# rust-bio/rust-bio

Measured on NVIDIA H100. Metric: GCUPS, higher is better.
Workload: dtype int32

## Files before the change

### rust_bio_b200/csrc/b2a_kernels.cuh

```cuda
#pragma once
#include <cuda_runtime.h>

#include "b2a_common.cuh"

namespace b2a {

struct PackParams {
  const Block* blocks;
  const uint32_t* order;
  const uint8_t* blob;
  const uint64_t* x_off;
  const uint32_t* x_len;
  const uint64_t* y_off;
  const uint32_t* y_len;
  const uint8_t* codemap;
  uint8_t* seq;
  uint32_t* bad_symbol;
  int32_t G;
  int32_t mapped;
};

__global__ void __launch_bounds__(256) pack_kernel(const PackParams prm) {
  __shared__ uint8_t cmap[256];
  __shared__ uint64_t s_off[64];
  __shared__ uint32_t s_len[64];
  cmap[threadIdx.x] = prm.codemap[threadIdx.x];
  const Block blk = prm.blocks[blockIdx.x];
  if (threadIdx.x < 64) {
    const uint32_t pair = threadIdx.x & 31u;
    const bool isy = threadIdx.x >= 32;
    uint64_t off = 0;
    uint32_t len = 0;
    if (pair < blk.npairs) {
      const uint32_t orig = prm.order[blk.first + pair];
      off = isy ? prm.y_off[orig] : prm.x_off[orig];
      len = isy ? prm.y_len[orig] : prm.x_len[orig];
    }
    s_off[threadIdx.x] = off;
    s_len[threadIdx.x] = len;
  }
  __syncthreads();
  const int G = prm.G, P = 32 / G;
  uint32_t* out = reinterpret_cast<uint32_t*>(prm.seq + blk.seq_off);
  const uint32_t xtot = blk.xwords * 32, ytot = blk.ywords * 32;
  for (uint32_t k = threadIdx.x; k < xtot + ytot; k += blockDim.x) {
    const bool isy = k >= xtot;
    const uint32_t kk = isy ? k - xtot : k;
    const uint32_t words = isy ? blk.ywords : blk.xwords;
    const uint32_t pair = kk / words, w = kk % words;
    uint32_t val = 0;
    {
      const uint64_t off = s_off[pair + (isy ? 32u : 0u)];
      const uint32_t len = s_len[pair + (isy ? 32u : 0u)];
      const uint32_t pos0 = w * 4;
      if (pos0 < len) {
        uint32_t raw;
        const uint32_t have = len - pos0 < 4 ? len - pos0 : 4;
        if (((off & 3ull) == 0) && have == 4) {
          raw = *reinterpret_cast<const uint32_t*>(prm.blob + off + pos0);
        } else {
          raw = 0;
          for (uint32_t b = 0; b < have; ++b) raw |= (uint32_t)prm.blob[off + pos0 + b] << (8 * b);
        }
#pragma unroll
        for (int b = 0; b < 4; ++b) {
          if ((uint32_t)b < have) {
            uint32_t code = cmap[(raw >> (8 * b)) & 0xFFu];
            if (prm.mapped && code == 0xFFu) {
              *prm.bad_symbol = 1u;
              code = 0;
            }
            val |= code << (8 * b);
          }
        }
      }
    }
    const uint32_t sub = pair / P, p = pair % P;
    out[(isy ? (size_t)G * blk.xwords * P : 0) + ((size_t)sub * words + w) * P + p] = val;
  }
}

__global__ void __launch_bounds__(256) symbols_kernel(const uint8_t* __restrict__ blob, uint64_t n,
                                                      uint32_t* __restrict__ flags) {
  __shared__ uint32_t seen[256];
  seen[threadIdx.x] = 0;
  __syncthreads();
  const uint64_t stride = (uint64_t)gridDim.x * blockDim.x;
  for (uint64_t i = blockIdx.x * (uint64_t)blockDim.x + threadIdx.x; i < n; i += stride) seen[blob[i]] = 1u;
  __syncthreads();
  if (seen[threadIdx.x]) flags[threadIdx.x] = 1u;
}

__global__ void gather_ops_kernel(const uint8_t* __restrict__ scratch,
                                  const uint64_t* __restrict__ ops_src,
                                  const uint64_t* __restrict__ ops_off, uint8_t* __restrict__ dense,
                                  uint64_t n_pairs) {
  const uint64_t warp = (blockIdx.x * (uint64_t)blockDim.x + threadIdx.x) >> 5;
  const uint32_t lane = threadIdx.x & 31;
  if (warp >= n_pairs) return;
  const uint64_t lo = ops_off[warp], n = ops_off[warp + 1] - lo;
  const uint8_t* src = scratch + ops_src[warp];
  for (uint64_t k = lane; k < n; k += 32) dense[lo + k] = src[k];
}

__global__ void __launch_bounds__(1024) scan_small_kernel(const uint32_t* __restrict__ n_ops, uint64_t* __restrict__ off,
                                                          uint32_t n_pairs) {
  __shared__ uint32_t wsum[64][32];
  __shared__ uint32_t round_tot[64];
  __shared__ uint64_t round_base[65];
  const uint32_t lane = threadIdx.x & 31u, w = threadIdx.x >> 5;
  const uint32_t rounds = (n_pairs + 1023u) >> 10;
  auto warp_inc = [&](uint32_t v) {
    for (int d = 1; d < 32; d <<= 1) {
      const uint32_t t = __shfl_up_sync(0xffffffffu, v, d);
      if (lane >= (uint32_t)d) v += t;
    }
    return v;
  };
  for (uint32_t k = 0; k < rounds; ++k) {
    const uint32_t i = (k << 10) + threadIdx.x;
    const uint32_t inc = warp_inc(i < n_pairs ? n_ops[i] : 0u);
    if (lane == 31) wsum[k][w] = inc;
  }
  __syncthreads();
  for (uint32_t k = w; k < rounds; k += 32) {
    const uint32_t ws = wsum[k][lane], wi = warp_inc(ws);
    wsum[k][lane] = wi - ws;
    if (lane == 31) round_tot[k] = wi;
  }
  __syncthreads();
  if (w == 0) {
    uint64_t carry = 0;
    for (uint32_t k0 = 0; k0 < rounds; k0 += 32) {
      const uint32_t k = k0 + lane;
      const uint64_t v = k < rounds ? (uint64_t)round_tot[k] : 0ull;
      uint64_t inc = v;
      for (int d = 1; d < 32; d <<= 1) {
        const uint64_t t = __shfl_up_sync(0xffffffffu, inc, d);
        if (lane >= (uint32_t)d) inc += t;
      }
      if (k < rounds) round_base[k] = carry + inc - v;
      carry += __shfl_sync(0xffffffffu, inc, 31);
    }
    if (lane == 0) round_base[rounds] = carry;
  }
  __syncthreads();
  for (uint32_t k = 0; k < rounds; ++k) {
    const uint32_t i = (k << 10) + threadIdx.x;
    const uint32_t v = i < n_pairs ? n_ops[i] : 0u;
    const uint32_t inc = warp_inc(v);
    if (i < n_pairs) off[i] = round_base[k] + wsum[k][w] + (inc - v);
  }
  if (threadIdx.x == 0) off[n_pairs] = round_base[rounds];
}

__global__ void widen_kernel(const uint32_t* __restrict__ n_ops, uint64_t* __restrict__ out,
                             uint64_t n_pairs) {
  const uint64_t i = blockIdx.x * (uint64_t)blockDim.x + threadIdx.x;
  if (i <= n_pairs) out[i] = i < n_pairs ? n_ops[i] : 0;
}

__global__ void records_kernel(const int32_t* score, const uint32_t* xstart, const uint32_t* xend,
                               const uint32_t* ystart, const uint32_t* yend, const uint32_t* n_ops,
                               const uint32_t* clip_len, const uint8_t* scratch,
                               const uint64_t* ops_src, uint8_t* records, uint32_t stride,
                               uint64_t n_pairs) {
  const uint64_t warp = (blockIdx.x * (uint64_t)blockDim.x + threadIdx.x) >> 5;
  const uint32_t lane = threadIdx.x & 31;
  if (warp >= n_pairs) return;
  uint8_t* rec = records + warp * stride;
  uint32_t* head = reinterpret_cast<uint32_t*>(rec);
  const uint32_t n = n_ops[warp];
  if (lane == 0) {
    head[0] = (uint32_t)score[warp];
    head[1] = xstart[warp];
    head[2] = xend[warp];
    head[3] = ystart[warp];
    head[4] = yend[warp];
    head[5] = n;
  }
  if (lane < 4) head[6 + lane] = clip_len[4 * warp + lane];
  const uint8_t* src = scratch + ops_src[warp];
  for (uint32_t k = lane; k < stride - 40; k += 32) rec[40 + k] = k < n ? src[k] : 0;
}

}
```

Before: 852.7.

## Transpose pack_kernel output through a padded shared-memory tile for coalesced stores

```diff
diff --git a/rust_bio_b200/csrc/b2a_kernels.cuh b/rust_bio_b200/csrc/b2a_kernels.cuh
--- a/rust_bio_b200/csrc/b2a_kernels.cuh
+++ b/rust_bio_b200/csrc/b2a_kernels.cuh
@@ -20,10 +20,40 @@
   int32_t mapped;
 };
 
+__device__ __forceinline__ uint32_t pack_word(const PackParams& prm, const uint8_t* cmap, const uint64_t off,
+                                              const uint32_t len, const uint32_t w) {
+  uint32_t val = 0;
+  const uint32_t pos0 = w * 4;
+  if (pos0 < len) {
+    uint32_t raw;
+    const uint32_t have = len - pos0 < 4 ? len - pos0 : 4;
+    if (((off & 3ull) == 0) && have == 4) {
+      raw = *reinterpret_cast<const uint32_t*>(prm.blob + off + pos0);
+    } else {
+      raw = 0;
+      for (uint32_t b = 0; b < have; ++b) raw |= (uint32_t)prm.blob[off + pos0 + b] << (8 * b);
+    }
+#pragma unroll
+    for (int b = 0; b < 4; ++b) {
+      if ((uint32_t)b < have) {
+        uint32_t code = cmap[(raw >> (8 * b)) & 0xFFu];
+        if (prm.mapped && code == 0xFFu) {
+          *prm.bad_symbol = 1u;
+          code = 0;
+        }
+        val |= code << (8 * b);
+      }
+    }
+  }
+  return val;
+}
+
+constexpr int PACK_CW_LOG = 6, PACK_CW = 1 << PACK_CW_LOG;
 __global__ void __launch_bounds__(256) pack_kernel(const PackParams prm) {
   __shared__ uint8_t cmap[256];
   __shared__ uint64_t s_off[64];
   __shared__ uint32_t s_len[64];
+  __shared__ uint32_t tile[PACK_CW * 33];
   cmap[threadIdx.x] = prm.codemap[threadIdx.x];
   const Block blk = prm.blocks[blockIdx.x];
   if (threadIdx.x < 64) {
@@ -41,42 +71,23 @@
   }
   __syncthreads();
   const int G = prm.G, P = 32 / G;
-  uint32_t* out = reinterpret_cast<uint32_t*>(prm.seq + blk.seq_off);
-  const uint32_t xtot = blk.xwords * 32, ytot = blk.ywords * 32;
-  for (uint32_t k = threadIdx.x; k < xtot + ytot; k += blockDim.x) {
-    const bool isy = k >= xtot;
-    const uint32_t kk = isy ? k - xtot : k;
-    const uint32_t words = isy ? blk.ywords : blk.xwords;
-    const uint32_t pair = kk / words, w = kk % words;
-    uint32_t val = 0;
-    {
-      const uint64_t off = s_off[pair + (isy ? 32u : 0u)];
-      const uint32_t len = s_len[pair + (isy ? 32u : 0u)];
-      const uint32_t pos0 = w * 4;
-      if (pos0 < len) {
-        uint32_t raw;
-        const uint32_t have = len - pos0 < 4 ? len - pos0 : 4;
-        if (((off & 3ull) == 0) && have == 4) {
-          raw = *reinterpret_cast<const uint32_t*>(prm.blob + off + pos0);
-        } else {
-          raw = 0;
-          for (uint32_t b = 0; b < have; ++b) raw |= (uint32_t)prm.blob[off + pos0 + b] << (8 * b);
-        }
-#pragma unroll
-        for (int b = 0; b < 4; ++b) {
-          if ((uint32_t)b < have) {
-            uint32_t code = cmap[(raw >> (8 * b)) & 0xFFu];
-            if (prm.mapped && code == 0xFFu) {
-              *prm.bad_symbol = 1u;
-              code = 0;
-            }
-            val |= code << (8 * b);
-          }
-        }
+  const int plog = 31 - __clz(P);
+  for (int side = 0; side < 2; ++side) {
+    const uint32_t words = side ? blk.ywords : blk.xwords;
+    uint32_t* out = reinterpret_cast<uint32_t*>(prm.seq + blk.seq_off) + (side ? (size_t)G * blk.xwords * P : 0);
+    for (uint32_t w0 = 0; w0 < words; w0 += PACK_CW) {
+      const uint32_t cw = words - w0 < (uint32_t)PACK_CW ? words - w0 : (uint32_t)PACK_CW;
+      for (uint32_t k = threadIdx.x; k < 32u * PACK_CW; k += blockDim.x) {
+        const uint32_t pair = k >> PACK_CW_LOG, wl = k & (PACK_CW - 1);
+        if (wl < cw) tile[wl * 33 + pair] = pack_word(prm, cmap, s_off[32 * side + pair], s_len[32 * side + pair], w0 + wl);
       }
+      __syncthreads();
+      for (uint32_t k = threadIdx.x; k < 32u * PACK_CW; k += blockDim.x) {
+        const uint32_t p = k & (P - 1), wl = (k >> plog) & (PACK_CW - 1), sub = k >> (plog + PACK_CW_LOG);
+        if (wl < cw) out[((size_t)sub * words + w0 + wl) * P + p] = tile[wl * 33 + sub * P + p];
+      }
+      __syncthreads();
     }
-    const uint32_t sub = pair / P, p = pair % P;
-    out[(isy ? (size_t)G * blk.xwords * P : 0) + ((size_t)sub * words + w) * P + p] = val;
   }
 }
 
```

Result: faster. 876.0, median of 6 (+2.7%).
